# vbruder/VolumeRendererCL

Measured on AMD Instinct MI355X. Metric: Msamples/s (samples taken, rays x steps after ESS/ERT) at 1024x1024 viewport, 2048^3 UCHAR, higher is better.
Workload: dtype f32; 1 GPU; shells2048: 2048^3 UCHAR 'shells' field generated in HBM, 1024x1024 viewport (launch grid 1032x1032), view rot30, TF default, illumType 1, object-order ESS on, ERT 0.98, samplingRate 1.5, per-frame mt19937 jitter seeds

## Files before the change

### include/vrhip.h

```cpp
#ifndef VRHIP_H
#define VRHIP_H

#include <stddef.h>
#include <stdint.h>

#ifdef __cplusplus
extern "C" {
#endif

#define VRHIP_ABI_VERSION 1

enum vrhip_status {
    VRHIP_OK = 0,
    VRHIP_ERR_INVALID = 1,
    VRHIP_ERR_HIP = 2,
    VRHIP_ERR_NODATA = 3,
    VRHIP_ERR_UNSUPPORTED = 4
};

enum vrhip_format { VRHIP_UCHAR = 0, VRHIP_USHORT = 1, VRHIP_FLOAT = 2 };

typedef struct vrhip_camera_params {
    float viewMat[16];
    float bbox_bl[4];
// ... 165 lines not shown
    uint32_t phase1_waves;
    uint32_t phase2_waves;
    uint32_t round_budget;
    uint32_t footprint;
    uint32_t empty_skip;
    uint32_t skip_in_lds;
    uint32_t instrumented;
    uint32_t extras;
    uint32_t patch_classes;
    uint32_t sorted_phase2;
    uint32_t views;
    uint32_t samples;
    uint32_t reserved[14];
    uint32_t pixel_major;
} vrhip_launch_info;
int vrhip_last_launch_info(const vrhip_renderer *r, vrhip_launch_info *out);

int vrhip_download_cost_map(vrhip_renderer *r, uint16_t *out, size_t n);

int vrhip_download_ray_order(vrhip_renderer *r, uint32_t sizes[8], uint32_t *out_items, size_t n_items,
                             uint32_t *out_notes, size_t n_notes, uint32_t out_counters[16], uint32_t *out_records,
                             size_t n_records, uint32_t *out_index, size_t n_index);

int vrhip_set_stats_enabled(vrhip_renderer *r, int enabled);
int vrhip_get_stats(const vrhip_renderer *r, vrhip_stats *out);
int vrhip_count_touched(vrhip_renderer *r, uint32_t width, uint32_t height,
                        uint64_t *microbricks_touched, uint8_t *bitmap_host, size_t bitmap_bytes);
int vrhip_count_fetched(vrhip_renderer *r, uint32_t width, uint32_t height, uint64_t *microbricks_fetched);
int vrhip_count_touched_tiles(vrhip_renderer *r, uint32_t width, uint32_t height,
                              uint32_t tile_w, uint32_t tile_h, const uint32_t *tile_ids,
                              uint32_t n_tiles, uint64_t *microbricks_touched);

const char *vrhip_build_source_hash(void);

#ifdef __cplusplus
}
#endif
#endif
```

### volumerenderercl_amd/_lib.py

```python
import ctypes as C
import os

_HERE = os.path.dirname(os.path.abspath(__file__))
LIB_PATH = os.environ.get("VRHIP_LIB_PATH") or os.path.join(_HERE, "libvrhip.so")

OK, ERR_INVALID, ERR_HIP, ERR_NODATA, ERR_UNSUPPORTED = range(5)
UCHAR, USHORT, FLOAT = 0, 1, 2
TECH_RAYCAST, TECH_PATHTRACE, TECH_MIP = 0, 1, 2
TECH_ISO = 4


class CameraParams(C.Structure):
    _fields_ = [("viewMat", C.c_float * 16), ("bbox_bl", C.c_float * 4),
                ("bbox_tr", C.c_float * 4), ("ortho", C.c_uint32), ("_pad", C.c_uint32 * 7)]


class RenderingParams(C.Structure):
    _fields_ = [("backgroundColor", C.c_float * 4), ("modelScale", C.c_float * 4),
                ("illumType", C.c_uint32), ("imgEss", C.c_uint32), ("showEss", C.c_uint32),
                ("useLinear", C.c_uint32), ("useGradient", C.c_uint32),
                ("technique", C.c_uint32), ("seed", C.c_uint32), ("iteration", C.c_uint32)]


class RaycastParams(C.Structure):
# ... 92 lines not shown
    "vrhip_build_bricks": (C.c_int, [_H]),
    "vrhip_get_brick_info": (C.c_int, [_H, _U3, C.POINTER(C.c_float), _U3]),
    "vrhip_download_bricks": (C.c_int, [_H, C.c_uint32, C.c_void_p, C.c_size_t]),
    "vrhip_last_bricks_seconds": (C.c_double, [_H]),
    "vrhip_set_camera_params": (C.c_int, [_H, C.POINTER(CameraParams)]),
    "vrhip_set_rendering_params": (C.c_int, [_H, C.POINTER(RenderingParams)]),
    "vrhip_set_raycast_params": (C.c_int, [_H, C.POINTER(RaycastParams)]),
    "vrhip_set_pathtrace_params": (C.c_int, [_H, C.POINTER(PathtraceParams)]),
    "vrhip_set_iso_params": (C.c_int, [_H, C.POINTER(IsoParams)]),
    "vrhip_set_object_ess": (C.c_int, [_H, C.c_int]),
    "vrhip_render_frame": (C.c_int, [_H, C.c_uint32, C.c_uint32, C.c_void_p, C.c_int]),
    "vrhip_render_tiles": (C.c_int, [_H, C.c_uint32, C.c_uint32, C.c_uint32, C.c_uint32,
                                     C.c_void_p, C.c_uint32, C.c_void_p]),
    "vrhip_set_environment_map": (C.c_int, [_H, C.c_void_p, C.c_uint32, C.c_uint32]),
    "vrhip_reset_image_ess": (C.c_int, [_H]),
    "vrhip_get_image_ess": (C.c_int, [_H, C.c_uint32, C.c_uint32, C.c_void_p, C.c_void_p]),
    "vrhip_set_image_ess": (C.c_int, [_H, C.c_uint32, C.c_uint32, C.c_void_p, C.c_void_p]),
    "vrhip_last_kernel_seconds": (C.c_double, [_H]),
    "vrhip_last_phase_seconds": (C.c_int, [_H, C.POINTER(C.c_double), C.POINTER(C.c_double)]),
    "vrhip_last_launch_info": (C.c_int, [_H, C.POINTER(LaunchInfo)]),
    "vrhip_download_cost_map": (C.c_int, [_H, C.c_void_p, C.c_size_t]),
    "vrhip_download_ray_order": (C.c_int, [_H, C.POINTER(C.c_uint32), C.c_void_p, C.c_size_t, C.c_void_p, C.c_size_t,
                                           C.POINTER(C.c_uint32), C.c_void_p, C.c_size_t, C.c_void_p, C.c_size_t]),
    "vrhip_set_phase_timing": (C.c_int, [_H, C.c_int]),
    "vrhip_set_frame_timing": (C.c_int, [_H, C.c_int]),
    "vrhip_build_source_hash": (C.c_char_p, []),
    "vrhip_set_stats_enabled": (C.c_int, [_H, C.c_int]),
    "vrhip_get_stats": (C.c_int, [_H, C.POINTER(Stats)]),
    "vrhip_count_touched": (C.c_int, [_H, C.c_uint32, C.c_uint32, C.POINTER(C.c_uint64),
                                      C.c_void_p, C.c_size_t]),
    "vrhip_count_fetched": (C.c_int, [_H, C.c_uint32, C.c_uint32, C.POINTER(C.c_uint64)]),
    "vrhip_count_touched_tiles": (C.c_int, [_H, C.c_uint32, C.c_uint32, C.c_uint32, C.c_uint32,
                                            C.c_void_p, C.c_uint32, C.POINTER(C.c_uint64)]),
}

_lib = None


def load():
    global _lib
    if _lib is not None:
        return _lib
    if not os.path.exists(LIB_PATH):
        raise RuntimeError(
            "libvrhip.so is not built (%s missing). Build it with "
            "`make -C volumerenderercl_amd/csrc` or __graft_entry__.build(); there is no "
# ... 11 lines not shown
```

### volumerenderercl_amd/csrc/vr_internal.h

```cpp
#pragma once
#include <hip/hip_runtime.h>
#include <hip/hip_ext.h>
#include <stdint.h>

#include <cstdio>
#include <cstdlib>
#include <map>
#include <mutex>
#include <tuple>
#include <utility>

#include "../../include/vrhip.h"

struct VolView {
    const void *data;
    int w, h, d;
    float fw, fh, fd;
    float inv_max;
    uint32_t nbx, nby, nbz;
    uint32_t ystride;
    unsigned long long zstride;
    const void *chan[3];
    int channels;
    const void *fp;
// ... 204 lines not shown
        last(bind_stop ? a.stop_event : nullptr);
        e = hipGetLastError();
    }
    if (e == hipSuccess && bind_stop) *a.stop_bound = true;
    return e;
}

template <typename VT>
struct VoxelType {
    using type = VT;
};
template <typename F>
inline hipError_t vr_for_format(int format, F f)
{
    switch (format) {
    case VRHIP_UCHAR: return f(VoxelType<uint8_t>());
    case VRHIP_USHORT: return f(VoxelType<uint16_t>());
    case VRHIP_FLOAT: return f(VoxelType<float>());
    default: return hipErrorInvalidValue;
    }
}

hipError_t vr_launch_raycast(const RaycastLaunch &a, hipStream_t stream);
hipError_t vr_launch_patch_classes(const RaycastLaunch &a, uint32_t n_patches, uint32_t set_frames, uint8_t *cls,
                                   hipStream_t stream);
hipError_t vr_launch_build_footprint(const VolView &vol, int format, hipStream_t stream);
hipError_t vr_launch_pathtrace(const RaycastLaunch &a, hipStream_t stream);
inline size_t vr_cell_record_bytes(int format) { return format == VRHIP_UCHAR ? 2 : format == VRHIP_USHORT ? 4 : 8; }
hipError_t vr_launch_cell_minmax(const VolView &vol, int format, const CellView &grid,
                                 float2 *minmax, hipStream_t stream, void *records = nullptr);
hipError_t vr_launch_cell_bounds(const float2 *minmax, const CellView &grid, float inv_max,
                                 const TfView &tf, float *sparse_scratch, float *bound,
                                 uint32_t *empty_bits, hipStream_t stream);
hipError_t vr_launch_cell_reduce(const float2 *fine, const CellView &grid, float2 *coarse, hipStream_t stream);
#ifndef VR_LEAP_SHIFT
#define VR_LEAP_SHIFT 2
#endif
constexpr int kLeapShift = VR_LEAP_SHIFT;
hipError_t vr_launch_cell_coarse_bounds(const CellView &grid, float *cbound, hipStream_t stream);
constexpr int kLeapLevels = 7, kLeapRadius = 15;
hipError_t vr_launch_cell_leap_radius(const CellView &grid, const float *cbound, uint8_t *dist, const uint8_t **result,
                                      hipStream_t stream);
hipError_t vr_launch_mip(const RaycastLaunch &a, hipStream_t stream);
hipError_t vr_launch_iso(const RaycastLaunch &a, hipStream_t stream);
inline hipError_t vr_launch_frame(const RaycastLaunch &a, hipStream_t stream)
{
    return a.render.technique == VRHIP_TECHNIQUE_ISO   ? vr_launch_iso(a, stream)
           : a.render.technique == VRHIP_TECHNIQUE_MIP ? vr_launch_mip(a, stream)
// ... 48 lines not shown
```

### volumerenderercl_amd/csrc/vr_raycast.hip

```cpp
#include "vr_raycast_kernels.h"

namespace {

__global__ __launch_bounds__(kBlockDim) void vr_patch_class_kernel(SkipView skip, FrameView fr, vrhip_camera_params cam,
                                                                   vrhip_rendering_params rp, Grid grid,
                                                                   uint32_t n_patches, uint32_t set_frames, uint8_t *cls)
{
    const uint32_t lane = threadIdx.x & 63u;
    const uint32_t pi = blockIdx.x * (kBlockDim / 64) + (threadIdx.x >> 6);
    if (pi >= n_patches) return;
    const WaveTile wt = fr.queue[(size_t)pi * set_frames];
    const float *V = cam.viewMat;
    const f3 ms = mk3(rp.modelScale[0], rp.modelScale[1], rp.modelScale[2]);
    const int maxImg = (int)(fr.gsx > fr.gsy ? fr.gsx : fr.gsy);
    const float spanx = (float)(11u + ((uint32_t)maxImg + fr.gsx - 1u) / fr.gsx);
    const float spany = (float)(11u + ((uint32_t)maxImg + fr.gsy - 1u) / fr.gsy);
    const float fx = (float)(wt_col(wt) * 8u) - 2.f + (float)(lane & 7u) * (spanx / 7.f);
    const float fy = (float)(wt_row(wt) * 8u) - 2.f + (float)(lane >> 3) * (spany / 7.f);
    float icx = (fx / (float)maxImg) * 2.f, icy = (fy / (float)maxImg) * 2.f;
    if (fr.gsx > fr.gsy) { icx -= 1.0f; icy -= fr.ray_aspect; }
    else { icx -= fr.ray_aspect; icy -= 1.0f; }
    icy *= -1.f;
    f3 npp = mk3(icx, icy, -1.0f);
    f3 rayDir = mk3(dot3(mk3(V[0], V[1], V[2]), npp), dot3(mk3(V[4], V[5], V[6]), npp), dot3(mk3(V[8], V[9], V[10]), npp));
    f3 camPos = mul3(mk3(V[3], V[7], V[11]), ms);
    if (cam.ortho) {
        camPos = mk3(V[3], V[7], V[11]);
        rayDir = neg3(mk3(V[2], V[6], V[10]));
        npp = add3(add3(camPos, scale3(mk3(V[0], V[4], V[8]), icx)), scale3(mk3(V[1], V[5], V[9]), icy));
        npp = scale3(npp, len3(camPos));
        camPos = mul3(npp, ms);
    }
    rayDir = normalize3(mul3(rayDir, ms));
    const float o[3] = {camPos.x, camPos.y, camPos.z}, dv[3] = {rayDir.x, rayDir.y, rayDir.z};
    float tn = -3.0e38f, tf = 3.0e38f, tns = -3.0e38f, tfs = 3.0e38f;
    for (int i = 0; i < 3; ++i) {
        const float inv = 1.0f / dv[i];
        const float m = 1.0e-3f * (cam.bbox_tr[i] - cam.bbox_bl[i]);
        const float tb = inv * (cam.bbox_bl[i] - o[i]), tt = inv * (cam.bbox_tr[i] - o[i]);
        const float tbs = inv * (cam.bbox_bl[i] + m - o[i]), tts = inv * (cam.bbox_tr[i] - m - o[i]);
        tn = vmax(tn, vmin(tt, tb)); tf = vmin(tf, vmax(tt, tb));
        tns = vmax(tns, vmin(tts, tbs)); tfs = vmin(tfs, vmax(tts, tbs));
    }
    const bool hit_shrunk = (tfs > tns) && !(tfs < 0.f) && (tfs - tns) > 0.f;
    RayCtx c;
    c.cam = camPos;
    c.dir = rayDir;
    c.valid = (tf > tn) && !(tf < 0.f);
    c.tnear = vmax(0.f, tn);
    c.tfar = tf;
    const bool inside = wt_col(wt) * 8u + 8u <= fr.W && wt_row(wt) * 8u + 8u <= fr.H;
    const bool all_hit = __ballot(hit_shrunk) == ~0ull;
    bool clear = false;
    if (inside && all_hit && skip.near_bits) clear = patch_is_clear(skip, grid, c, lane);
    if (lane == 0) cls[pi] = clear ? 1 : 0;
}


__global__ __launch_bounds__(kBlockDim) void vr_regroup_kernel(FrameView fr, uint32_t group)
{
    const uint32_t lane = threadIdx.x & 63u;
    const uint32_t n = fr.n_wave_tiles, sf = fr.set_frames;
    const uint32_t p = blockIdx.x * (kBlockDim / 64) + (threadIdx.x >> 6);
    if (p >= n / sf) return;
    const uint32_t *notes = fr.pm + 2u * (size_t)p * sf;
    const uint32_t *first = fr.pm + 2u * (size_t)n + (size_t)p * sf;
    uint32_t total = 0;
    for (uint32_t f0 = 0; f0 < sf; f0 += 64u) {
        const uint32_t f = f0 + lane;
        const uint32_t c = f < sf ? (uint32_t)(__builtin_popcount(notes[2u * f]) + __builtin_popcount(notes[2u * f + 1u])) : 0u;
        total += (uint32_t)wave_sum((unsigned long long)c);
    }
    total = __builtin_amdgcn_readfirstlane(total);
    if (!total) return;
    const uint32_t padded = (total + group - 1u) & ~(group - 1u);
    const uint32_t list = p % kLiveLists;
    uint32_t base = 0;
    if (lane == 0) base = atomicAdd(fr.live_list_count + (kPmBase - kLiveBase) + list * kLiveStride, padded);
// ... 205 lines not shown
    case VRHIP_USHORT:
        hipLaunchKernelGGL(vr_skipmap_kernel<uint16_t>, grid, block, 0, stream, bricks, inv_max, tf,
                           bits, n_words);
        break;
    case VRHIP_FLOAT:
        hipLaunchKernelGGL(vr_skipmap_kernel<float>, grid, block, 0, stream, bricks, inv_max, tf,
                           bits, n_words);
        break;
    default: return hipErrorInvalidValue;
    }
    return hipGetLastError();
}

hipError_t vr_launch_regroup(const FrameView &frame, uint32_t group, hipStream_t stream)
{
    if (!frame.pm || !frame.set_frames || (group != 1u && group != 32u && group != 64u)) return hipErrorInvalidValue;
    const uint32_t n_patches = frame.n_wave_tiles / frame.set_frames;
    if (!n_patches) return hipSuccess;
    hipLaunchKernelGGL(vr_regroup_kernel, dim3((n_patches + kBlockDim / 64 - 1u) / (kBlockDim / 64)), dim3(kBlockDim), 0, stream, frame, group);
    return hipGetLastError();
}

hipError_t vr_launch_patch_classes(const RaycastLaunch &a, uint32_t n_patches, uint32_t set_frames, uint8_t *cls,
                                   hipStream_t stream)
{
    if (!n_patches) return hipSuccess;
    const Grid hg = make_grid_host(a);
    hipLaunchKernelGGL(vr_patch_class_kernel, dim3((n_patches + 3u) / 4u), dim3(kBlockDim), 0, stream, a.skip, a.frame,
                       a.cam, a.render, hg, n_patches, set_frames, cls);
    return hipGetLastError();
}
```

### volumerenderercl_amd/csrc/vr_raycast_kernels.h

```cpp
#pragma once
#include <algorithm>
#include <vector>

#include "vr_sampling.h"

hipError_t vr_launch_raycast_u8(const RaycastLaunch &a, hipStream_t stream);
hipError_t vr_launch_raycast_u16(const RaycastLaunch &a, hipStream_t stream);
hipError_t vr_launch_raycast_f32(const RaycastLaunch &a, hipStream_t stream);
hipError_t vr_launch_cont_sort(const FrameView &frame, hipStream_t stream);
hipError_t vr_launch_regroup(const FrameView &frame, uint32_t group, hipStream_t stream);
#if defined(VR_MARCH_STATS) || defined(VR_STAMPS)
enum { VR_DEBUG_MARCH_STATS = 0, VR_DEBUG_STAMPS = 1, VR_DEBUG_WAVE_SPAN = 2 };
int vr_raycast_debug_int(int which, unsigned long long *sum, size_t n, int reset);
int vr_raycast_debug_f32(int which, unsigned long long *sum, size_t n, int reset);
#endif

namespace {

constexpr int kSplit = 4;

#ifdef VR_MARCH_STATS
__device__ unsigned long long g_march_stats[32];
#define VR_MS(i, v) ms_acc[i] += (unsigned long long)(v)
#else
#define VR_MS(i, v)
#endif
#ifdef VR_ISA_MARKS
#define VR_MARK(x) asm volatile("; VRMARK " x ::: "memory")
#else
#define VR_MARK(x)
#endif

#ifdef VR_WAVES_PER_EU
#define VR_OCC __attribute__((amdgpu_waves_per_eu(VR_WAVES_PER_EU, VR_WAVES_PER_EU)))
#else
#define VR_OCC
#endif

struct RayCtx {
    f3 cam, dir;
    float env0, env1, env2, env3;
    float tnear;
    float tfar, sampleDist, stepSize, offset;
    f3 lgt, hv;
    bool hvalid;
    int stepv0, stepv1, stepv2, exit0, exit1, exit2;
    float dT0, dT1, dT2;
    bool valid;
// ... 913 lines not shown
        const float p[3] = {rc.x + t * rd.x, rc.y + t * rd.y, rc.z + t * rd.z};
        int cell[3];
        for (int i = 0; i < 3; ++i) cell[i] = iclamp((int)floorf((p[i] + 1.f) * ibs[i]), 0, bres[i] - 1);
        const uint32_t idx = ((uint32_t)cell[2] * (uint32_t)g.bh + (uint32_t)cell[1]) * (uint32_t)g.bw + (uint32_t)cell[0];
        live = live || ((skip.near_bits[idx >> 5] >> (idx & 31u)) & 1u);
    }
    return __ballot(live) == 0ull;
}


template <typename VT, bool VIEWS = false>
__global__ __launch_bounds__(kBlockDim) void vr_dda_prepass_kernel(
    VolView vv, BrickView bricks, SkipView skip, FrameView fr, vrhip_camera_params cam,
    vrhip_rendering_params rp, vrhip_raycast_params rc, Grid grid, f3 voxLen)
{
    VR_ZERO_NEXT_CTRL(fr);
    const uint32_t lane = threadIdx.x & 63u;
    const uint32_t q = blockIdx.x * (kBlockDim / 64) + (threadIdx.x >> 6);
    if (q >= fr.n_wave_tiles) return;
    const WaveTile wt = fr.queue[q];
    const uint32_t lx = lane & 7u, ly = lane >> 3;
    const uint32_t gx = wt_col(wt) * 8u + lx, gy = wt_row(wt) * 8u + ly;
    const size_t out_index = (size_t)wt.out_base + (size_t)ly * fr.out_stride + lx;
    if (fr.patch_class && fr.patch_class[q / fr.set_frames]) {
        const float4 o = make_float4(rp.backgroundColor[0], rp.backgroundColor[1], rp.backgroundColor[2], 0.f);
        fr.fb[(size_t)gy * fr.W + gx] = o;
        if (fr.out) fr.out[out_index] = o;
        VR_PM_NOTE(fr, q, 0ull, 0u);
        return;
    }
    const uint32_t seed = fr.seeds ? fr.seeds[wt_frame(wt)] : rp.seed;
    const bool inside = gx < fr.W && gy < fr.H;
    const f3 resf = mk3(vv.fw, vv.fh, vv.fd);
    RayCtx c;
    RayDyn d;
    float rnd;
    if constexpr (VIEWS) {
        const vrhip_camera_params fc = load_frame_cam<true>(fr.cams, wt_frame(wt));
        setup_ray_head<false>(gx, gy, inside, fr, fc, rp, c, d, seed, rnd);
    } else {
        setup_ray_head<false>(gx, gy, inside, fr, cam, rp, c, d, seed, rnd);
    }
    if (rp.imgEss && image_ess_patch(fr, rp, c, wt, lane, inside, gx, gy, out_index)) {
        VR_PM_NOTE(fr, q, 0ull, 0u);
        return;
    }
    if (skip.near_bits && patch_is_clear(skip, grid, c, lane)) {
        if (inside) write_pixel<true>(fr, rp, c, d, voxLen, gx, gy, out_index);
        VR_PM_NOTE(fr, q, 0ull, 0u);
        return;
    }
    setup_ray_tail<true>(rc, resf, voxLen, grid, c, d, rnd);
    fetch_skip_word(skip.bits, grid, d);
    unsigned long long n0 = 0, n1 = 0;
#ifdef VR_MARCH_STATS
    unsigned long long w_steps = 0, l_steps = 0;
    while (__ballot(d.state == S_BRICK)) {
        w_steps++;
        l_steps += __builtin_popcountll(__ballot(d.state == S_BRICK));
        dda_step<0>(skip.bits, grid, c, d, n0, n1);
    }
    if (lane == 0) {
        atomicAdd(&g_march_stats[28], 1ull);
        atomicAdd(&g_march_stats[29], w_steps);
        atomicAdd(&g_march_stats[30], l_steps);
        atomicAdd(&g_march_stats[31], (unsigned long long)__builtin_popcountll(__ballot(c.valid)));
    }
#else
    while (__ballot(d.state == S_BRICK)) dda_step<0>(skip.bits, grid, c, d, n0, n1);
#endif
    const bool live = d.state == S_SAMPLE;
    const unsigned long long m = __ballot(live);
    if (inside && !live) {
        write_pixel<true>(fr, rp, c, d, voxLen, gx, gy, out_index);
    }
    if (fr.live_rays) {
        if (m) {
            const uint32_t list = q % kLiveLists;
            VR_WAVE_APPEND(base, fr.live_list_count + list * kLiveStride, m);
            base += list * live_list_cap(fr.n_wave_tiles);
            VR_PM_NOTE(fr, q, m, base);
            if (live) {
                VR_PACK_RAY(r, (uint32_t)out_index, wt_frame(wt), 0);
                fr.live_rays[base + VR_LANE_RANK(m)] = r;
            }
        } else {
            VR_PM_NOTE(fr, q, 0ull, 0u);
        }
        return;
    }
    if (m && lane == 0) {
        const uint32_t slot = atomicAdd(fr.live_count, 1u);
        LiveTile lt;
        lt.wt = wt;
        lt.mask_lo = (uint32_t)m;
// ... 703 lines not shown
```

### volumerenderercl_amd/csrc/vr_renderer.h

```cpp
#ifndef VR_RENDERER_H
#define VR_RENDERER_H

#include <hip/hip_runtime.h>

#include <cstring>
#include <string>
#include <vector>

#include "vr_internal.h"

template <class T = void>
struct DevBuf {
    T *p = nullptr;
    size_t bytes = 0;
    bool owned = true;

    DevBuf() = default;
    DevBuf(const DevBuf &) = delete;
    DevBuf &operator=(const DevBuf &) = delete;
    DevBuf(DevBuf &&o) noexcept : p(o.p), bytes(o.bytes), owned(o.owned) { o.forget(); }
    DevBuf &operator=(DevBuf &&o) noexcept
    {
        if (this != &o) {
            release();
// ... 101 lines not shown

    vrhip_camera_params cam;
    vrhip_rendering_params render;
    vrhip_raycast_params raycast;
    vrhip_pathtrace_params pathtrace;
    vrhip_iso_params iso;
    bool use_ess = true;

    DevBuf<float4> fb;
    uint32_t fb_w = 0, fb_h = 0;

    DevBuf<DevStats> stats_dev;
    bool stats_enabled = false;

    DevBuf<WaveTile> queue_dev;
    uint32_t queue_n = 0;
    DevBuf<uint32_t> queue_head;
    DevBuf<uint8_t> patch_class;
    std::vector<uint8_t> patch_class_key;
    uint32_t skip_version = 0;
    uint32_t queue_version = 0;
    uint32_t queue_frames = 1;
    bool use_patch_classes = true;
    int occ_force = 0;
    int occ_force_split = 0;
    uint32_t ctrl_sel = 0;
    bool ctrl_clean[2] = {false, false};
    bool phase_timing = false;
    int event_bind = 2;
    bool frame_timing = true;
    DevBuf<uint16_t> cost;
    DevBuf<uint32_t> order;
    DevBuf<ContRec> live_rays;
    bool ray_list = true;
    DevBuf<uint32_t> pm;
    bool pixel_major = true;
    uint32_t pm_group = 64;
    bool pm_last = false;
    uint32_t pm_last_ctrl = 0, pm_last_frames = 0;
    DevBuf<uint32_t> seeds_dev;
    DevBuf<vrhip_camera_params> cams_dev;
    DevBuf<> samples_dev;
    bool sort_cont = true;
    DevBuf<LiveTile> live;
    bool prepass = true;
    DevBuf<ContRec> cont;
// ... 260 lines not shown
```

### volumerenderercl_amd/csrc/vrhip_api.hip

```cpp
#include <hip/hip_runtime.h>

#include <algorithm>
#include <cmath>
#include <cstdio>
#include <cstdlib>
#include <cstring>
#include <string>
#include <vector>

#include "vr_renderer.h"

namespace {

constexpr uint32_t kSkipLdsMaxBytes = 64 * 1024;
constexpr uint32_t kDefaultSamplesPerLaunch = 64;
constexpr unsigned long long kDefaultSampleRecords = 64ull << 20;

size_t volume_bytes(const vrhip_renderer *r)
{
    return (size_t)r->res[0] * r->res[1] * r->res[2] * fmt_bytes(r->format);
}

size_t volume_alloc_bytes(const vrhip_renderer *r)
{
// ... 531 lines not shown
    a->num_cus = r->num_cus;
}

int ensure_patch_classes(vrhip_renderer *r, RaycastLaunch *a)
{
    a->frame.patch_class = nullptr;
    a->frame.set_frames = r->queue_frames;
    const vrhip_rendering_params &rp = a->render;
    if (!r->use_patch_classes || a->frame.cams || rp.technique != 0 || !a->use_ess || a->instr != 0 || !a->frame.live || !a->skip.near_bits ||
        rp.useGradient || a->frame.env || rp.showEss || rp.imgEss || rp.iteration != 0)
        return VRHIP_OK;
    const uint32_t n_patches = r->queue_n / r->queue_frames;
    std::vector<uint8_t> key;
    auto put = [&key](const void *p, size_t n) { key.insert(key.end(), (const uint8_t *)p, (const uint8_t *)p + n); };
    vrhip_rendering_params rk = rp;
    rk.seed = 0;
    put(&a->cam, sizeof a->cam);
    put(&rk, sizeof rk);
    put(&a->raycast, sizeof a->raycast);
    const uint32_t misc[10] = {a->frame.W, a->frame.H, a->frame.gsx, a->frame.gsy, r->queue_version, r->skip_version,
                               a->skip.near_r, n_patches, r->queue_frames, (uint32_t)a->bricks.bw};
    put(misc, sizeof misc);
    if (key != r->patch_class_key) {
        const int rc = grow(r, r->patch_class, n_patches);
        if (rc) return rc;
        r->patch_class_key.clear();
        VR_HIP(r, vr_launch_patch_classes(*a, n_patches, r->queue_frames, r->patch_class, r->stream));
        r->patch_class_key.swap(key);
        if (getenv("VRHIP_DEBUG")) {
            std::vector<uint8_t> h(n_patches);
            VR_HIP(r, hipMemcpyAsync(h.data(), r->patch_class, n_patches, hipMemcpyDeviceToHost, r->stream));
            VR_HIP(r, hipStreamSynchronize(r->stream));
            size_t n1 = 0;
            for (uint8_t v : h) n1 += v;
            fprintf(stderr, "[vrhip] patch classes: %zu of %u patches are background for every jitter\n", n1, n_patches);
        }
    }
    a->frame.patch_class = r->patch_class;
    return VRHIP_OK;
}

int launch_timed(vrhip_renderer *r, const RaycastLaunch &a)
{
    if (a.instr && !a.keep_stats) VR_HIP(r, hipMemsetAsync(r->stats_dev, 0, sizeof(DevStats), r->stream));
    if (!r->ctrl_clean[r->ctrl_sel])
        VR_HIP(r, hipMemsetAsync(a.frame.queue_head, 0, kControlWords * sizeof(uint32_t), r->stream));
    r->ctrl_clean[r->ctrl_sel] = false;
    RaycastLaunch b = a;
    {
        const int rc = ensure_patch_classes(r, &b);
        if (rc) return rc;
    }
    bool start_bound = false, stop_bound = false;
    b.bind_events = r->event_bind;
    if (r->frame_timing) {
        b.stop_event = r->ev1;
        b.stop_bound = &stop_bound;
        if (r->event_bind >= 2) {
// ... 152 lines not shown
        return fail(nullptr, VRHIP_ERR_HIP, msg);
    }
    r->stream = r->own_stream;
    if (getenv("VRHIP_MARCH") || getenv("VRHIP_LDS_STAGE") || getenv("VRHIP_MARCH_MICRO")) {
        vrhip_destroy(r);
        return fail(nullptr, VRHIP_ERR_UNSUPPORTED,
                    "VRHIP_MARCH / VRHIP_LDS_STAGE / VRHIP_MARCH_MICRO: the VR_EXPERIMENTS kernels were removed "
                    "(commit 858be18 holds them)");
    }
    if (const char *b = getenv("VRHIP_ROUND_BUDGET")) r->round_budget = (uint32_t)atoi(b);
    if (getenv("VRHIP_NO_PREPASS")) r->prepass = false;
    if (getenv("VRHIP_NO_RAYLIST")) r->ray_list = false;
    if (const char *e = getenv("VRHIP_CULL_RADIUS")) {
        const int v = atoi(e);
        if (v >= 0 && v <= 64) r->cull_radius = (uint32_t)v;
    }
    if (getenv("VRHIP_NO_SORT")) r->sort_cont = false;
    if (const char *e = getenv("VRHIP_PIXEL_MAJOR")) r->pixel_major = atoi(e) != 0;
    if (const char *e = getenv("VRHIP_PM_GROUP")) {
        const int v = atoi(e);
        if (v == 1 || v == 32 || v == 64) r->pm_group = (uint32_t)v;
    }
    if (getenv("VRHIP_NO_PATCH_CLASS")) r->use_patch_classes = false;
    auto occ_env = [](const char *name, int dflt) {
        const char *e = getenv(name);
        return e ? (atoi(e) == 3 ? 3 : atoi(e) == 2 ? 2 : 0) : dflt;
    };
    if (const char *e = getenv("VRHIP_FRAME_TIMING")) r->frame_timing = atoi(e) != 0;
    if (const char *e = getenv("VRHIP_EVENT_BIND")) r->event_bind = atoi(e);
    r->occ_force = r->occ_force_split = occ_env("VRHIP_OCC", 0);
    r->occ_force = occ_env("VRHIP_OCC_P1", r->occ_force);
    r->occ_force_split = occ_env("VRHIP_OCC_P2", r->occ_force_split);
    if (getenv("VRHIP_PT_NO_CULL")) r->pt_cull = false;
    if (getenv("VRHIP_PT_NO_LEAP")) r->pt_leap = false;
    if (getenv("VRHIP_PT_NO_FAR_LEAP")) r->pt_leap_far = false;
    if (getenv("VRHIP_NO_EMPTY_SKIP")) r->skip_empty = false;
    if (getenv("VRHIP_EMPTY_SKIP")) r->skip_empty_force = true;
    if (getenv("VRHIP_NO_FOOTPRINT")) r->use_fp = false;
    if (const char *e = getenv("VRHIP_REFILL_MIN")) {
        const int v = atoi(e);
        if (v >= 1 && v <= 16) r->refill_min = (uint32_t)v;
    }
    if (const char *e = getenv("VRHIP_INGEST_SLAB_BYTES")) {
        const unsigned long long v = strtoull(e, nullptr, 10);
        if (v > 0) r->ingest_slab_bytes = (size_t)v;
    }
// ... 652 lines not shown
    if (phase2) *phase2 = (double)b * 1e-3;
    return VRHIP_OK;
}

int vrhip_last_launch_info(const vrhip_renderer *r, vrhip_launch_info *out)
{
    if (!r || !out) return VRHIP_ERR_INVALID;
    if (!r->have_info) return fail(r, VRHIP_ERR_NODATA, "vrhip_last_launch_info: nothing has been rendered yet");
    *out = r->last_info;
    return VRHIP_OK;
}

int vrhip_download_cost_map(vrhip_renderer *r, uint16_t *out, size_t n)
{
    if (!r || !out) return VRHIP_ERR_INVALID;
    if (set_device(r)) return VRHIP_ERR_HIP;
    VR_REQUIRE(r, r->cost && n == (size_t)r->fb_w * r->fb_h, VRHIP_ERR_NODATA,
               "vrhip_download_cost_map: no cost map of this size (render a frame first)");
    VR_HIP(r, hipStreamSynchronize(r->stream));
    VR_HIP(r, hipMemcpy(out, r->cost, n * sizeof(uint16_t), hipMemcpyDeviceToHost));
    return VRHIP_OK;
}

int vrhip_download_ray_order(vrhip_renderer *r, uint32_t sizes[8], uint32_t *out_items, size_t n_items,
                             uint32_t *out_notes, size_t n_notes, uint32_t out_counters[16], uint32_t *out_records,
                             size_t n_records, uint32_t *out_index, size_t n_index)
{
    if (!r) return VRHIP_ERR_INVALID;
    if (set_device(r)) return VRHIP_ERR_HIP;
    VR_REQUIRE(r, r->pm_last && r->pm && r->live_rays && r->queue_dev && r->queue_head, VRHIP_ERR_NODATA,
               "vrhip_download_ray_order: the last render call was not a launch set in pixel-major order");
    const uint32_t n = r->queue_n, sf = r->pm_last_frames;
    const uint32_t ray_cap = live_list_cap(n), idx_cap = pm_list_cap(n, sf);
    VR_HIP(r, hipStreamSynchronize(r->stream));
    std::vector<uint32_t> ctrl(kControlWords);
    VR_HIP(r, hipMemcpy(ctrl.data(), r->queue_head + (size_t)r->pm_last_ctrl * kControlWords, kControlWords * sizeof(uint32_t),
                        hipMemcpyDeviceToHost));
    uint32_t counters[2 * kLiveLists], take[2 * kLiveLists];
    size_t n_rec = 0, n_ent = 0;
    for (uint32_t k = 0; k < kLiveLists; ++k) {
        counters[k] = ctrl[kLiveBase + k * kLiveStride];
        counters[kLiveLists + k] = ctrl[kPmBase + k * kLiveStride];
        take[k] = counters[k] < ray_cap ? counters[k] : ray_cap;
        take[kLiveLists + k] = counters[kLiveLists + k] < idx_cap ? counters[kLiveLists + k] : idx_cap;
        n_rec += take[k];
        n_ent += take[kLiveLists + k];
// ... 169 lines not shown
```

### volumerenderercl_amd/renderer.py

```python
import ctypes as C

import numpy as np

from . import _lib, frontend
from ._lib import (CameraParams, IsoParams, PathtraceParams, RaycastParams, RenderingParams, Stats,
                   UCHAR, USHORT, FLOAT, TECH_MIP, TECH_ISO)

NP_DTYPE = {UCHAR: np.uint8, USHORT: np.uint16, FLOAT: np.float32}
_MT19937_DEFAULT_SEED = 5489


def _u3(v):
    return (C.c_uint32 * 3)(*[int(x) for x in v])


class VolumeRenderCL:
    TECH_RAYCAST, TECH_PATHTRACE = 0, 1

    def __init__(self):
        self._lib = None
        self._h = C.c_void_p()
        self._vol_loaded = False
        self._model_scale = np.ones(3, dtype=np.float32)
        self._camera = CameraParams()
# ... 626 lines not shown
    def downloadRayOrder(self):
        fn = self._lib.vrhip_download_ray_order
        sizes, counters = (C.c_uint32 * 8)(), (C.c_uint32 * 16)()
        self._check(fn(self._h, sizes, None, 0, None, 0, counters, None, 0, None, 0))
        sf, n, group, ray_cap, idx_cap, n_rec, n_ent = (int(v) for v in sizes[:7])
        items = np.empty((n, 3), dtype=np.uint32)
        notes = np.empty(3 * n, dtype=np.uint32)
        recs = np.empty((n_rec, 4), dtype=np.uint32)
        ents = np.empty(n_ent, dtype=np.uint32)
        self._check(fn(self._h, sizes, items.ctypes.data_as(C.c_void_p), items.size, notes.ctypes.data_as(C.c_void_p),
                       notes.size, counters, recs.ctypes.data_as(C.c_void_p), recs.size, ents.ctypes.data_as(C.c_void_p),
                       ents.size))
        ray_counts = [int(v) for v in counters[:8]]
        index_counts = [int(v) for v in counters[8:]]
        rcut = np.cumsum([0] + [min(c, ray_cap) for c in ray_counts])
        icut = np.cumsum([0] + [min(c, idx_cap) for c in index_counts])
        ballot = notes[0:2 * n:2].astype(np.uint64) | (notes[1:2 * n:2].astype(np.uint64) << np.uint64(32))
        return {"set_frames": sf, "n_items": n, "group": group, "live_list_cap": ray_cap, "pm_list_cap": idx_cap,
                "items": items.astype(np.int64), "notes": notes, "ballot": ballot, "first": notes[2 * n:].astype(np.int64),
                "ray_counts": ray_counts, "index_counts": index_counts,
                "records": [recs[rcut[k]:rcut[k + 1]].astype(np.int64) for k in range(8)],
                "index": [ents[icut[k]:icut[k + 1]].copy() for k in range(8)]}

    def setSeed(self, seed):
        self._fixed_seed = None if seed is None else int(seed) & 0xFFFFFFFF
        if self._fixed_seed is not None:
            self._rendering.seed = self._fixed_seed

    def setIteration(self, it):
        self._rendering.iteration = int(it)

    def setStatsEnabled(self, v):
        self._check(self._lib.vrhip_set_stats_enabled(self._h, 1 if v else 0))

    def getStats(self):
        st = Stats()
        self._check(self._lib.vrhip_get_stats(self._h, C.byref(st)))
        return st.as_dict()

    def countTouched(self, width, height, want_bitmap=False):
        n = C.c_uint64()
        bm = None
        if want_bitmap:
            mb = [(r + 3) // 4 for r in self._res[:3]]
            bm = np.zeros((mb[0] * mb[1] * mb[2] + 7) // 8, dtype=np.uint8)
        self._push_params()
# ... 29 lines not shown
```

Baseline: 195,200 Msamples/s.

## Add brick-splat coverage and grown-box miss tests to patch classification

Extends the per-patch prepass in two ways. A new splat kernel projects each non-empty brick's padded bounds to screen space and sets a coverage bitmap of 8x8 patches. Patches no brick reaches are marked clear, and patches whose rays all miss a box grown by the jitter spread become a background class. The raycast kernel then writes background directly for these patches and skips ray setup and marching. The cost is an extra splat kernel with atomics, a memset, and more prepass arithmetic, and the conservative bounds could misclassify patches if they are too tight. It also adds a debug download API and stats counters.

```diff
diff --git a/include/vrhip.h b/include/vrhip.h
--- a/include/vrhip.h
+++ b/include/vrhip.h
@@ -211,6 +211,9 @@
                              uint32_t *out_notes, size_t n_notes, uint32_t out_counters[16], uint32_t *out_records,
                              size_t n_records, uint32_t *out_index, size_t n_index);
 
+int vrhip_download_patch_classes(vrhip_renderer *r, uint32_t *n_patches, uint8_t *out, size_t n, uint32_t *out_items,
+                                 size_t n_items);
+
 int vrhip_set_stats_enabled(vrhip_renderer *r, int enabled);
 int vrhip_get_stats(const vrhip_renderer *r, vrhip_stats *out);
 int vrhip_count_touched(vrhip_renderer *r, uint32_t width, uint32_t height,
diff --git a/volumerenderercl_amd/_lib.py b/volumerenderercl_amd/_lib.py
--- a/volumerenderercl_amd/_lib.py
+++ b/volumerenderercl_amd/_lib.py
@@ -138,6 +138,7 @@
     "vrhip_download_cost_map": (C.c_int, [_H, C.c_void_p, C.c_size_t]),
     "vrhip_download_ray_order": (C.c_int, [_H, C.POINTER(C.c_uint32), C.c_void_p, C.c_size_t, C.c_void_p, C.c_size_t,
                                            C.POINTER(C.c_uint32), C.c_void_p, C.c_size_t, C.c_void_p, C.c_size_t]),
+    "vrhip_download_patch_classes": (C.c_int, [_H, C.POINTER(C.c_uint32), C.c_void_p, C.c_size_t, C.c_void_p, C.c_size_t]),
     "vrhip_set_phase_timing": (C.c_int, [_H, C.c_int]),
     "vrhip_set_frame_timing": (C.c_int, [_H, C.c_int]),
     "vrhip_build_source_hash": (C.c_char_p, []),
diff --git a/volumerenderercl_amd/csrc/vr_internal.h b/volumerenderercl_amd/csrc/vr_internal.h
--- a/volumerenderercl_amd/csrc/vr_internal.h
+++ b/volumerenderercl_amd/csrc/vr_internal.h
@@ -250,8 +250,10 @@
 }
 
 hipError_t vr_launch_raycast(const RaycastLaunch &a, hipStream_t stream);
+inline uint32_t patch_cover_wpr(uint32_t W) { return ((W + 7u) / 8u + 31u) / 32u; }
+inline uint32_t patch_cover_words(uint32_t W, uint32_t H) { return ((H + 7u) / 8u) * patch_cover_wpr(W); }
 hipError_t vr_launch_patch_classes(const RaycastLaunch &a, uint32_t n_patches, uint32_t set_frames, uint8_t *cls,
-                                   hipStream_t stream);
+                                   uint32_t *cover, uint32_t mode, hipStream_t stream);
 hipError_t vr_launch_build_footprint(const VolView &vol, int format, hipStream_t stream);
 hipError_t vr_launch_pathtrace(const RaycastLaunch &a, hipStream_t stream);
 inline size_t vr_cell_record_bytes(int format) { return format == VRHIP_UCHAR ? 2 : format == VRHIP_USHORT ? 4 : 8; }
diff --git a/volumerenderercl_amd/csrc/vr_raycast.hip b/volumerenderercl_amd/csrc/vr_raycast.hip
--- a/volumerenderercl_amd/csrc/vr_raycast.hip
+++ b/volumerenderercl_amd/csrc/vr_raycast.hip
@@ -4,7 +4,9 @@
 
 __global__ __launch_bounds__(kBlockDim) void vr_patch_class_kernel(SkipView skip, FrameView fr, vrhip_camera_params cam,
                                                                    vrhip_rendering_params rp, Grid grid,
-                                                                   uint32_t n_patches, uint32_t set_frames, uint8_t *cls)
+                                                                   uint32_t n_patches, uint32_t set_frames, uint8_t *cls,
+                                                                   const uint32_t *cover, uint32_t cover_wpr,
+                                                                   uint32_t cover_words, uint32_t mode)
 {
     const uint32_t lane = threadIdx.x & 63u;
     const uint32_t pi = blockIdx.x * (kBlockDim / 64) + (threadIdx.x >> 6);
@@ -33,16 +35,41 @@
     }
     rayDir = normalize3(mul3(rayDir, ms));
     const float o[3] = {camPos.x, camPos.y, camPos.z}, dv[3] = {rayDir.x, rayDir.y, rayDir.z};
-    float tn = -3.0e38f, tf = 3.0e38f, tns = -3.0e38f, tfs = 3.0e38f;
+    float rho = 0.f;
+    if (mode >= 2u) {
+        const int la = (int)((lane + 9u) & 63u), lb = (int)((lane + 1u) & 63u), lc = (int)((lane + 8u) & 63u);
+        const f3 ca = mk3(__shfl(camPos.x, la, 64), __shfl(camPos.y, la, 64), __shfl(camPos.z, la, 64));
+        const f3 cb = mk3(__shfl(camPos.x, lb, 64), __shfl(camPos.y, lb, 64), __shfl(camPos.z, lb, 64));
+        const f3 cc = mk3(__shfl(camPos.x, lc, 64), __shfl(camPos.y, lc, 64), __shfl(camPos.z, lc, 64));
+        const f3 da = mk3(__shfl(rayDir.x, la, 64), __shfl(rayDir.y, la, 64), __shfl(rayDir.z, la, 64));
+        const f3 db = mk3(__shfl(rayDir.x, lb, 64), __shfl(rayDir.y, lb, 64), __shfl(rayDir.z, lb, 64));
+        const f3 dc3 = mk3(__shfl(rayDir.x, lc, 64), __shfl(rayDir.y, lc, 64), __shfl(rayDir.z, lc, 64));
+        const bool cell = (lane & 7u) < 7u && lane < 56u;
+        const float dc = wave_max_f(cell ? vmax(len3(sub3(camPos, ca)), len3(sub3(cb, cc))) : 0.f);
+        const float dd = wave_max_f(cell ? vmax(len3(sub3(rayDir, da)), len3(sub3(db, dc3))) : 0.f);
+        float far2 = 0.f;
+        for (int k = 0; k < 8; ++k) {
+            const f3 p = mk3((k & 1) ? cam.bbox_tr[0] : cam.bbox_bl[0], (k & 2) ? cam.bbox_tr[1] : cam.bbox_bl[1],
+                             (k & 4) ? cam.bbox_tr[2] : cam.bbox_bl[2]);
+            far2 = vmax(far2, len3(sub3(p, camPos)));
+        }
+        const float T = wave_max_f(far2) + dc;
+        rho = (dc + T * dd) * 1.0001f;
+    }
+    float tn = -3.0e38f, tf = 3.0e38f, tns = -3.0e38f, tfs = 3.0e38f, tng = -3.0e38f, tfg = 3.0e38f;
     for (int i = 0; i < 3; ++i) {
         const float inv = 1.0f / dv[i];
         const float m = 1.0e-3f * (cam.bbox_tr[i] - cam.bbox_bl[i]);
+        const float g = m + 1.25f * rho;
         const float tb = inv * (cam.bbox_bl[i] - o[i]), tt = inv * (cam.bbox_tr[i] - o[i]);
         const float tbs = inv * (cam.bbox_bl[i] + m - o[i]), tts = inv * (cam.bbox_tr[i] - m - o[i]);
+        const float tbg = inv * (cam.bbox_bl[i] - g - o[i]), ttg = inv * (cam.bbox_tr[i] + g - o[i]);
         tn = vmax(tn, vmin(tt, tb)); tf = vmin(tf, vmax(tt, tb));
         tns = vmax(tns, vmin(tts, tbs)); tfs = vmin(tfs, vmax(tts, tbs));
+        tng = vmax(tng, vmin(ttg, tbg)); tfg = vmin(tfg, vmax(ttg, tbg));
     }
     const bool hit_shrunk = (tfs > tns) && !(tfs < 0.f) && (tfs - tns) > 0.f;
+    const bool miss_grown = (tfg < tng) || (tfg < 0.f);
     RayCtx c;
     c.cam = camPos;
     c.dir = rayDir;
@@ -51,9 +78,79 @@
     c.tfar = tf;
     const bool inside = wt_col(wt) * 8u + 8u <= fr.W && wt_row(wt) * 8u + 8u <= fr.H;
     const bool all_hit = __ballot(hit_shrunk) == ~0ull;
+    const bool all_miss = mode >= 2u && rho < 1.0e30f && __ballot(miss_grown) == ~0ull;
     bool clear = false;
     if (inside && all_hit && skip.near_bits) clear = patch_is_clear(skip, grid, c, lane);
-    if (lane == 0) cls[pi] = clear ? 1 : 0;
+    if (!clear && inside && all_hit && mode >= 3u && cover && cover[cover_words] == 0u &&
+        skip.bits[skip.n_words] == 0xffffffffu) {
+        const uint32_t col = wt_col(wt), row = wt_row(wt);
+        clear = !((cover[(size_t)row * cover_wpr + (col >> 5)] >> (col & 31u)) & 1u);
+    }
+    if (lane == 0) cls[pi] = clear ? 1 : (inside && all_miss ? 2 : 0);
+}
+
+__global__ __launch_bounds__(kBlockDim) void vr_patch_splat_kernel(SkipView skip, FrameView fr, vrhip_camera_params cam,
+                                                                   vrhip_rendering_params rp, Grid grid, uint32_t *cover,
+                                                                   uint32_t cover_wpr, uint32_t cover_words)
+{
+    const size_t n = (size_t)grid.bw * grid.bh * grid.bd;
+    const size_t i = (size_t)blockIdx.x * kBlockDim + threadIdx.x;
+    if (i >= n) return;
+    if ((skip.bits[i >> 5] >> (i & 31u)) & 1u) return;
+    const int b[3] = {(int)(i % (size_t)grid.bw), (int)((i / (size_t)grid.bw) % (size_t)grid.bh),
+                      (int)(i / ((size_t)grid.bw * grid.bh))};
+    const float bl[3] = {grid.bl0, grid.bl1, grid.bl2};
+    float lo[3], hi[3];
+    for (int k = 0; k < 3; ++k) {
+        lo[k] = -1.f + (2.f * bl[k]) * (float)(b[k] - 2);
+        hi[k] = -1.f + (2.f * bl[k]) * (float)(b[k] + 3);
+    }
+    const float *V = cam.viewMat;
+    const float r00 = V[0], r01 = V[1], r02 = V[2], r10 = V[4], r11 = V[5], r12 = V[6], r20 = V[8], r21 = V[9], r22 = V[10];
+    const float c00 = r11 * r22 - r12 * r21, c01 = r12 * r20 - r10 * r22, c02 = r10 * r21 - r11 * r20;
+    const float idet = 1.f / (r00 * c00 + r01 * c01 + r02 * c02);
+    const f3 i0 = scale3(mk3(c00, r02 * r21 - r01 * r22, r01 * r12 - r02 * r11), idet);
+    const f3 i1 = scale3(mk3(c01, r00 * r22 - r02 * r20, r02 * r10 - r00 * r12), idet);
+    const f3 i2 = scale3(mk3(c02, r01 * r20 - r00 * r21, r00 * r11 - r01 * r10), idet);
+    const f3 c0 = mk3(V[3], V[7], V[11]);
+    const float l = len3(c0);
+    const f3 org = cam.ortho ? scale3(c0, l) : c0;
+    const int maxImg = (int)(fr.gsx > fr.gsy ? fr.gsx : fr.gsy);
+    const float offx = fr.gsx > fr.gsy ? 1.0f : fr.ray_aspect, offy = fr.gsx > fr.gsy ? fr.ray_aspect : 1.0f;
+    float xmin = 3.0e38f, xmax = -3.0e38f, ymin = 3.0e38f, ymax = -3.0e38f;
+    bool bad = false;
+    for (int k = 0; k < 8; ++k) {
+        const f3 P = mk3((k & 1) ? hi[0] : lo[0], (k & 2) ? hi[1] : lo[1], (k & 4) ? hi[2] : lo[2]);
+        const f3 w = sub3(mk3(P.x / rp.modelScale[0], P.y / rp.modelScale[1], P.z / rp.modelScale[2]), org);
+        const f3 q = mk3(dot3(i0, w), dot3(i1, w), dot3(i2, w));
+        float s = l;
+        if (!cam.ortho) {
+            s = -q.z;
+            if (!(s > 0.05f * (fabsf(q.x) + fabsf(q.y))) || !(s > 1.0e-3f * len3(q))) bad = true;
+        }
+        const float px = (q.x / s + offx) * (0.5f * (float)maxImg), py = (offy - q.y / s) * (0.5f * (float)maxImg);
+        if (!(fabsf(px) < 1.0e30f) || !(fabsf(py) < 1.0e30f)) bad = true;
+        xmin = vmin(xmin, px); xmax = vmax(xmax, px);
+        ymin = vmin(ymin, py); ymax = vmax(ymax, py);
+    }
+    if (bad) {
+        cover[cover_words] = 1u;
+        return;
+    }
+    const uint32_t pw = (fr.W + 7u) / 8u, ph = (fr.H + 7u) / 8u;
+    const float jx = (float)(((uint32_t)maxImg + fr.gsx - 1u) / fr.gsx), jy = (float)(((uint32_t)maxImg + fr.gsy - 1u) / fr.gsy);
+    const float x0f = floorf((xmin - jx - 2.f) * 0.125f), x1f = ceilf((xmax + 2.f) * 0.125f) - 1.f;
+    const float y0f = floorf((ymin - jy - 2.f) * 0.125f), y1f = ceilf((ymax + 2.f) * 0.125f) - 1.f;
+    if (x1f < 0.f || y1f < 0.f || x0f > (float)(pw - 1u) || y0f > (float)(ph - 1u)) return;
+    const uint32_t x0 = (uint32_t)vmax(x0f, 0.f), x1 = (uint32_t)vmin(x1f, (float)(pw - 1u));
+    const uint32_t y0 = (uint32_t)vmax(y0f, 0.f), y1 = (uint32_t)vmin(y1f, (float)(ph - 1u));
+    for (uint32_t y = y0; y <= y1; ++y)
+        for (uint32_t wd = x0 >> 5; wd <= (x1 >> 5); ++wd) {
+            const uint32_t a = wd == (x0 >> 5) ? (x0 & 31u) : 0u, e = wd == (x1 >> 5) ? (x1 & 31u) : 31u;
+            const uint32_t m = (0xffffffffu >> (31u - e)) & (0xffffffffu << a);
+            uint32_t *p = cover + (size_t)y * cover_wpr + wd;
+            if ((*p & m) != m) atomicOr(p, m);
+        }
 }
 
 
@@ -305,11 +402,20 @@
 }
 
 hipError_t vr_launch_patch_classes(const RaycastLaunch &a, uint32_t n_patches, uint32_t set_frames, uint8_t *cls,
-                                   hipStream_t stream)
+                                   uint32_t *cover, uint32_t mode, hipStream_t stream)
 {
     if (!n_patches) return hipSuccess;
     const Grid hg = make_grid_host(a);
+    const uint32_t wpr = patch_cover_wpr(a.frame.W), words = patch_cover_words(a.frame.W, a.frame.H);
+    const size_t n_bricks = (size_t)hg.bw * hg.bh * hg.bd;
+    if (mode < 3u || !n_bricks) cover = nullptr;
+    if (cover) {
+        hipError_t e = hipMemsetAsync(cover, 0, ((size_t)words + 1u) * sizeof(uint32_t), stream);
+        if (e != hipSuccess) return e;
+        hipLaunchKernelGGL(vr_patch_splat_kernel, dim3((unsigned)((n_bricks + kBlockDim - 1) / kBlockDim)), dim3(kBlockDim), 0,
+                           stream, a.skip, a.frame, a.cam, a.render, hg, cover, wpr, words);
+    }
     hipLaunchKernelGGL(vr_patch_class_kernel, dim3((n_patches + 3u) / 4u), dim3(kBlockDim), 0, stream, a.skip, a.frame,
-                       a.cam, a.render, hg, n_patches, set_frames, cls);
+                       a.cam, a.render, hg, n_patches, set_frames, cls, (const uint32_t *)cover, wpr, words, mode);
     return hipGetLastError();
 }
diff --git a/volumerenderercl_amd/csrc/vr_raycast_kernels.h b/volumerenderercl_amd/csrc/vr_raycast_kernels.h
--- a/volumerenderercl_amd/csrc/vr_raycast_kernels.h
+++ b/volumerenderercl_amd/csrc/vr_raycast_kernels.h
@@ -22,8 +22,10 @@
 #ifdef VR_MARCH_STATS
 __device__ unsigned long long g_march_stats[32];
 #define VR_MS(i, v) ms_acc[i] += (unsigned long long)(v)
+#define VR_PREPASS_OUTCOME(i) do { if (lane == 0) atomicAdd(&g_march_stats[i], 1ull); } while (0)
 #else
 #define VR_MS(i, v)
+#define VR_PREPASS_OUTCOME(i)
 #endif
 #ifdef VR_ISA_MARKS
 #define VR_MARK(x) asm volatile("; VRMARK " x ::: "memory")
@@ -983,11 +985,13 @@
     const uint32_t lx = lane & 7u, ly = lane >> 3;
     const uint32_t gx = wt_col(wt) * 8u + lx, gy = wt_row(wt) * 8u + ly;
     const size_t out_index = (size_t)wt.out_base + (size_t)ly * fr.out_stride + lx;
-    if (fr.patch_class && fr.patch_class[q / fr.set_frames]) {
-        const float4 o = make_float4(rp.backgroundColor[0], rp.backgroundColor[1], rp.backgroundColor[2], 0.f);
+    if (const uint32_t pcl = fr.patch_class ? fr.patch_class[q / fr.set_frames] : 0u) {
+        const float4 o = make_float4(rp.backgroundColor[0], rp.backgroundColor[1], rp.backgroundColor[2],
+                                     pcl == 1u ? 0.f : rp.backgroundColor[3] * 1.f);
         fr.fb[(size_t)gy * fr.W + gx] = o;
         if (fr.out) fr.out[out_index] = o;
         VR_PM_NOTE(fr, q, 0ull, 0u);
+        VR_PREPASS_OUTCOME(pcl == 1u ? 0 : 1);
         return;
     }
     const uint32_t seed = fr.seeds ? fr.seeds[wt_frame(wt)] : rp.seed;
@@ -1009,6 +1013,7 @@
     if (skip.near_bits && patch_is_clear(skip, grid, c, lane)) {
         if (inside) write_pixel<true>(fr, rp, c, d, voxLen, gx, gy, out_index);
         VR_PM_NOTE(fr, q, 0ull, 0u);
+        VR_PREPASS_OUTCOME(2);
         return;
     }
     setup_ray_tail<true>(rc, resf, voxLen, grid, c, d, rnd);
@@ -1032,6 +1037,7 @@
 #endif
     const bool live = d.state == S_SAMPLE;
     const unsigned long long m = __ballot(live);
+    VR_PREPASS_OUTCOME(m ? 5 : (__ballot(c.valid) ? 4 : 3));
     if (inside && !live) {
         write_pixel<true>(fr, rp, c, d, voxLen, gx, gy, out_index);
     }
diff --git a/volumerenderercl_amd/csrc/vr_renderer.h b/volumerenderercl_amd/csrc/vr_renderer.h
--- a/volumerenderercl_amd/csrc/vr_renderer.h
+++ b/volumerenderercl_amd/csrc/vr_renderer.h
@@ -147,6 +147,8 @@
     uint32_t queue_version = 0;
     uint32_t queue_frames = 1;
     bool use_patch_classes = true;
+    DevBuf<uint32_t> patch_cover;
+    uint32_t patch_class_mode = 3;
     int occ_force = 0;
     int occ_force_split = 0;
     uint32_t ctrl_sel = 0;
diff --git a/volumerenderercl_amd/csrc/vrhip_api.hip b/volumerenderercl_amd/csrc/vrhip_api.hip
--- a/volumerenderercl_amd/csrc/vrhip_api.hip
+++ b/volumerenderercl_amd/csrc/vrhip_api.hip
@@ -577,18 +577,26 @@
                                a->skip.near_r, n_patches, r->queue_frames, (uint32_t)a->bricks.bw};
     put(misc, sizeof misc);
     if (key != r->patch_class_key) {
-        const int rc = grow(r, r->patch_class, n_patches);
+        bool box_in_volume = true;
+        for (int i = 0; i < 3; ++i)
+            box_in_volume = box_in_volume && a->cam.bbox_bl[i] >= -1.f && a->cam.bbox_tr[i] <= 1.f;
+        const uint32_t mode = r->patch_class_mode >= 3u && !box_in_volume ? 2u : r->patch_class_mode;
+        int rc = grow(r, r->patch_class, n_patches);
+        if (!rc && mode >= 3u)
+            rc = grow(r, r->patch_cover, ((size_t)patch_cover_words(a->frame.W, a->frame.H) + 1u) * sizeof(uint32_t));
         if (rc) return rc;
         r->patch_class_key.clear();
-        VR_HIP(r, vr_launch_patch_classes(*a, n_patches, r->queue_frames, r->patch_class, r->stream));
+        VR_HIP(r, vr_launch_patch_classes(*a, n_patches, r->queue_frames, r->patch_class,
+                                          mode >= 3u ? (uint32_t *)r->patch_cover : nullptr, mode, r->stream));
         r->patch_class_key.swap(key);
         if (getenv("VRHIP_DEBUG")) {
             std::vector<uint8_t> h(n_patches);
             VR_HIP(r, hipMemcpyAsync(h.data(), r->patch_class, n_patches, hipMemcpyDeviceToHost, r->stream));
             VR_HIP(r, hipStreamSynchronize(r->stream));
-            size_t n1 = 0;
-            for (uint8_t v : h) n1 += v;
-            fprintf(stderr, "[vrhip] patch classes: %zu of %u patches are background for every jitter\n", n1, n_patches);
+            size_t n1 = 0, n2 = 0;
+            for (uint8_t v : h) { n1 += v == 1; n2 += v == 2; }
+            fprintf(stderr, "[vrhip] patch classes (mode %u): of %u patches %zu are class 1 (no brick to sample), %zu class 2 (no ray hits the box), for every jitter\n",
+                    r->patch_class_mode, n_patches, n1, n2);
         }
     }
     a->frame.patch_class = r->patch_class;
@@ -787,6 +795,10 @@
         if (v == 1 || v == 32 || v == 64) r->pm_group = (uint32_t)v;
     }
     if (getenv("VRHIP_NO_PATCH_CLASS")) r->use_patch_classes = false;
+    if (const char *e = getenv("VRHIP_PATCH_CLASS_MODE")) {
+        const int m = atoi(e);
+        if (m >= 1 && m <= 3) r->patch_class_mode = (uint32_t)m;
+    }
     auto occ_env = [](const char *name, int dflt) {
         const char *e = getenv(name);
         return e ? (atoi(e) == 3 ? 3 : atoi(e) == 2 ? 2 : 0) : dflt;
@@ -1485,6 +1497,30 @@
     return VRHIP_OK;
 }
 
+int vrhip_download_patch_classes(vrhip_renderer *r, uint32_t *n_patches_out, uint8_t *out, size_t n, uint32_t *out_items,
+                                 size_t n_items)
+{
+    if (!r) return VRHIP_ERR_INVALID;
+    if (set_device(r)) return VRHIP_ERR_HIP;
+    VR_REQUIRE(r, r->have_info && r->last_info.patch_classes && !r->patch_class_key.empty() && r->patch_class && r->queue_dev &&
+                      r->queue_frames, VRHIP_ERR_NODATA, "vrhip_download_patch_classes: the last render call used no patch classes");
+    const uint32_t n_patches = r->queue_n / r->queue_frames;
+    if (n_patches_out) *n_patches_out = n_patches;
+    VR_REQUIRE(r, (!out || n == n_patches) && (!out_items || n_items == 2 * (size_t)n_patches), VRHIP_ERR_INVALID,
+               "vrhip_download_patch_classes: size mismatch");
+    VR_HIP(r, hipStreamSynchronize(r->stream));
+    if (out && n_patches) VR_HIP(r, hipMemcpy(out, r->patch_class, n_patches, hipMemcpyDeviceToHost));
+    if (out_items && n_patches) {
+        std::vector<WaveTile> q(r->queue_n);
+        VR_HIP(r, hipMemcpy(q.data(), r->queue_dev, (size_t)r->queue_n * sizeof(WaveTile), hipMemcpyDeviceToHost));
+        for (uint32_t i = 0; i < n_patches; ++i) {
+            out_items[2 * (size_t)i] = wt_col(q[(size_t)i * r->queue_frames]);
+            out_items[2 * (size_t)i + 1] = wt_row(q[(size_t)i * r->queue_frames]);
+        }
+    }
+    return VRHIP_OK;
+}
+
 int vrhip_download_ray_order(vrhip_renderer *r, uint32_t sizes[8], uint32_t *out_items, size_t n_items,
                              uint32_t *out_notes, size_t n_notes, uint32_t out_counters[16], uint32_t *out_records,
                              size_t n_records, uint32_t *out_index, size_t n_index)
diff --git a/volumerenderercl_amd/renderer.py b/volumerenderercl_amd/renderer.py
--- a/volumerenderercl_amd/renderer.py
+++ b/volumerenderercl_amd/renderer.py
@@ -672,6 +672,16 @@
                 "records": [recs[rcut[k]:rcut[k + 1]].astype(np.int64) for k in range(8)],
                 "index": [ents[icut[k]:icut[k + 1]].copy() for k in range(8)]}
 
+    def downloadPatchClasses(self):
+        fn = self._lib.vrhip_download_patch_classes
+        n = C.c_uint32(0)
+        self._check(fn(self._h, C.byref(n), None, 0, None, 0))
+        cls = np.empty(n.value, dtype=np.uint8)
+        items = np.empty((n.value, 2), dtype=np.uint32)
+        self._check(fn(self._h, C.byref(n), cls.ctypes.data_as(C.c_void_p), cls.size, items.ctypes.data_as(C.c_void_p),
+                       items.size))
+        return cls, items.astype(np.int64)
+
     def setSeed(self, seed):
         self._fixed_seed = None if seed is None else int(seed) & 0xFFFFFFFF
         if self._fixed_seed is not None:
```

New measurement: 197,400 Msamples/s, median of 6. 1.1% higher.
